# showlab/EgoVLP

Hardware: NVIDIA H100
Metric: clips/sec, 16-frame TimeSformer-B + DistilBERT + EgoNCE training step (higher is better)
Workload: dtype bf16

## Files before the change

### egovlp_b200/_lib.py

```python
import ctypes as C
import os

_PKG = os.path.dirname(os.path.abspath(__file__))
LIB_PATH = os.environ.get("EGOVLP_B200_LIB") or os.path.join(_PKG, "lib", "libegovlp_b200.so")
_lib = None


class GemmEpilogue(C.Structure):
    _fields_ = [("bias", C.c_void_p), ("residual", C.c_void_p), ("aux", C.c_void_p), ("out", C.c_void_p),
                ("out2", C.c_void_p), ("ldr", C.c_longlong), ("ldaux", C.c_longlong), ("ldo", C.c_longlong),
                ("ldo2", C.c_longlong), ("out_mode", C.c_int), ("act", C.c_int), ("alpha", C.c_float),
                ("col_scale", C.c_float), ("col_scale_ncols", C.c_int), ("res_row_mod", C.c_int), ("colsum", C.c_void_p),
                ("colsum_a", C.c_void_p), ("drop_p", C.c_float), ("drop_site", C.c_uint), ("drop_seed", C.c_ulonglong),
                ("path_p", C.c_float), ("path_site", C.c_uint), ("path_rows", C.c_int)]


class EgovlpError(RuntimeError):
    pass


def lib():
    global _lib
    if _lib is None:
        if not os.path.exists(LIB_PATH):
            raise EgovlpError(f"{LIB_PATH} is missing: build it with `python -m egovlp_b200.build` "
                              "(there is no CPU / PyTorch fallback for the hot path)")
        _lib = C.CDLL(LIB_PATH)
        _lib.egovlp_last_error.restype = C.c_char_p
        _lib.egovlp_divided_attn_workspace_floats.restype = C.c_longlong
        _lib.egovlp_egonce_fused_workspace_floats.restype = C.c_longlong
        _lib.egovlp_narrow_linear_workspace_floats.restype = C.c_longlong
        _lib.egovlp_space_attn_long_workspace_floats.restype = C.c_longlong
    return _lib


_KERNELS_PER_CALL = {"egovlp_egonce_fused_max_g": 0, "egovlp_divided_attn_fwd": 2, "egovlp_divided_attn_bwd": 2, "egovlp_video_embed_bwd": 2,
                     "egovlp_nce_fwd": 2, "egovlp_dual_softmax": 2, "egovlp_cross_entropy_fwd": 2,
                     "egovlp_narrow_linear_bwd": 3, "egovlp_text_attn_long_bwd": 3, "egovlp_space_attn_long_fwd": 2,
                     "egovlp_space_attn_long_bwd": 4}
_launches = 0


def reset_launch_count():
    global _launches
    _launches = 0


def launch_count():
    return _launches


def call(name, *args):
    global _launches
    fn = getattr(lib(), name)
    rc = fn(*args)
    _launches += _KERNELS_PER_CALL.get(name, 1)
    if rc != 0:
        raise EgovlpError(f"{name} failed ({rc}): {lib().egovlp_last_error().decode()}")


def declared_symbols():
    import re
# ... 5 lines not shown
```

### egovlp_b200/csrc/attention.cu

```cuda
#include <stdlib.h>

#include "common.cuh"
#include "egovlp_b200.h"

namespace egovlp {

bool space_attn_wgmma_supported(int N);
int space_attn_fwd_wgmma(const void* qkv, void* out, float* lse, float* cls_part, int B, int T, int N, int H,
                         cudaStream_t st);

namespace {

constexpr int HD = 64;
constexpr int ROW_BYTES = 128;
constexpr float LOG2E = 1.4426950408889634f;

struct Geom {
  int B, H, T, N, S, D;
  int mode;
  int PG;
  int G;
  int NP;
  int NPAD;
  int gsize;
};

__device__ __forceinline__ int row_token(const Geom& G, int g, int r) {
  if (r == G.NP) return 0;
  if (r > G.NP) return -1;
  if (G.mode == 1) return 1 + g * G.N + r;
  const int j = r / G.T, f = r - j * G.T, n = g * G.PG + j;
  return n < G.N ? 1 + f * G.N + n : -1;
}

template <int RT>
__device__ __forceinline__ int row_token_x(const Geom& G, int g, int r, int sh) {
  if (RT == 0) return row_token(G, g, r);
  if (r == G.NP) return 0;
  if (r > G.NP) return -1;
  if (RT == 1) return 1 + g * G.N + r;
  const int n = g * G.PG + (r >> sh);
  return n < G.N ? 1 + (r & ((1 << sh) - 1)) * G.N + n : -1;
}

struct Smem {
  uint32_t q, k, v, dout;
  short* gid;
  float* lse;
  float* delta;
  uint32_t stage;
  uint32_t bar;
};

__device__ __forceinline__ bool pair_valid(int gq, int gk, bool first_group) {
  if (gq >= 0) return gk == gq || gk == -2;
  if (gq == -2) return gk >= 0 || (gk == -2 && first_group);
  return false;
}

__device__ __forceinline__ void tile_window(const Geom& G, int r0, int& lo, int& hi) {
  if (r0 <= G.NP && G.NP < r0 + 16) { lo = 0; hi = G.NP; return; }
  if (r0 > G.NP) { lo = 0; hi = 0; return; }
  lo = (r0 / G.gsize) * G.gsize;
  hi = min(G.NP, ((r0 + 15) / G.gsize + 1) * G.gsize);
}
__device__ __forceinline__ bool span_active(const Geom& G, int lo, int hi, int c0, int width) {
  return (c0 < hi && c0 + width > lo) || (c0 <= G.NP && G.NP < c0 + width);
}

// ... 843 lines not shown
      }
      const float2 lq = *reinterpret_cast<const float2*>(sm.lse + col);
      const float2 dq2 = *reinterpret_cast<const float2*>(sm.delta + col);
      const f32x2 nl = pk2(-lq.x, -lq.y), nd = pk2(-dq2.x, -dq2.y);
      float e0, e1, e2, e3;
      up2(fma2(pk2(st[j][0], st[j][1]), sc, nl), e0, e1);
      up2(fma2(pk2(st[j][2], st[j][3]), sc, nl), e2, e3);
      const float p0 = exp2f(e0), p1 = exp2f(e1), p2 = exp2f(e2), p3 = exp2f(e3);
      pf[p][jj * 2] = pack_bf16x2(p0, p1);
      pf[p][jj * 2 + 1] = pack_bf16x2(p2, p3);
      float d0, d1, d2, d3;
      up2(mul2(pk2(p0, p1), add2(pk2(dpt[j][0], dpt[j][1]), nd)), d0, d1);
      up2(mul2(pk2(p2, p3), add2(pk2(dpt[j][2], dpt[j][3]), nd)), d2, d3);
      dsf[p][jj * 2] = pack_bf16x2(d0, d1);
      dsf[p][jj * 2 + 1] = pack_bf16x2(d2, d3);
    }
  }
#pragma unroll
  for (int p = 0; p < NPR; ++p) {
    const uint32_t qb = sm.q + ch.base[p] * ROW_BYTES, db = sm.dout + ch.base[p] * ROW_BYTES;
#pragma unroll
    for (int dpi = 0; dpi < 4; ++dpi) {
      uint32_t bf[4];
      ldsm_x4_t(db + fo.a[dpi], bf);
      mma_bf16(dv[2 * dpi], pf[p], bf[0], bf[1]);
      mma_bf16(dv[2 * dpi + 1], pf[p], bf[2], bf[3]);
      ldsm_x4_t(qb + fo.a[dpi], bf);
      mma_bf16(dk[2 * dpi], dsf[p], bf[0], bf[1]);
      mma_bf16(dk[2 * dpi + 1], dsf[p], bf[2], bf[3]);
    }
  }
}

template <bool TIME, int NWARPS, int MINB>
__global__ void __launch_bounds__(NWARPS * 32, MINB)
fast_attn_bwd_kernel(const __grid_constant__ CUtensorMap tm_qkv, const __grid_constant__ CUtensorMap tm_do,
                     const bf16* __restrict__ qkv, const bf16* __restrict__ out, const bf16* __restrict__ dout,
                     const float* __restrict__ lse_in, bf16* __restrict__ dqkv, float* __restrict__ dcls, float q_scale,
                     Geom G, int sh) {
  extern __shared__ uint8_t smem_raw[];
  const uint32_t smem_base = (smem_u32(smem_raw) + 1023u) & ~1023u;
  uint8_t* smem_gen = smem_raw + (smem_base - smem_u32(smem_raw));
  int b, h, g;
  decode_block(G, b, h, g);
  Smem sm;
  load_group<true, false, false, false>(G, &tm_qkv, &tm_do, qkv, dout, b, h, g, smem_gen, smem_base, sm, NWARPS);
  constexpr int RT = TIME ? 2 : 1;

  const int warp = threadIdx.x >> 5, lane = threadIdx.x & 31;
  const int gq = lane >> 2, t = lane & 3;
  FastCtx c;
  c.NP = G.NP; c.NPAD = G.NPAD; c.sh = sh; c.first_group = (g == 0);
  c.valid_keys = TIME ? min(G.PG, G.N - g * G.PG) * G.T : G.NP;
  const FragOff fo = make_frag_off(lane);

  constexpr int P0_ROWS = NWARPS * 4;
  constexpr int P0_MAX = (256 + P0_ROWS - 1) / P0_ROWS;
  constexpr int P0_N = TIME ? 128 / P0_ROWS : P0_MAX;
  uint4 o_pre[P0_N];
  float l_pre[P0_N];
  int t_pre[P0_N];
#pragma unroll
  for (int i = 0; i < P0_N; ++i) {
    const int r = warp * 4 + (lane >> 3) + i * P0_ROWS;
    const int tok = r < G.NPAD ? row_token_x<RT>(G, g, r, sh) : -1;
    t_pre[i] = tok;
    const int tc = max(tok, 0);
    o_pre[i] = __ldg(reinterpret_cast<const uint4*>(out + ((long long)b * G.S + tc) * G.D + h * HD + (lane & 7) * 8));
    l_pre[i] = __ldg(lse_in + ((long long)(b * G.H + h)) * G.S + tc);
  }
  mbar_wait(sm.bar, 0);
#pragma unroll
  for (int i = 0; i < P0_N; ++i) {
    const int r = warp * 4 + (lane >> 3) + i * P0_ROWS;
    if (r >= G.NPAD) break;
    const int tok = t_pre[i], cc = lane & 7;
    float d = 0.f;
    if (tok >= 0) {
      const uint4 ov = o_pre[i];
      const uint4 dv = *reinterpret_cast<const uint4*>(smem_gen + (sw_addr(sm.dout, r, cc) - smem_base));
      const uint32_t ou[4] = {ov.x, ov.y, ov.z, ov.w}, du[4] = {dv.x, dv.y, dv.z, dv.w};
#pragma unroll
      for (int i = 0; i < 4; ++i) {
        const float2 a = unpack_bf16x2(ou[i]), bb = unpack_bf16x2(du[i]);
        d += a.x * bb.x + a.y * bb.y;
      }
    }
    d += __shfl_xor_sync(0xffffffffu, d, 1); d += __shfl_xor_sync(0xffffffffu, d, 2); d += __shfl_xor_sync(0xffffffffu, d, 4);
    if (cc == 0) {
      sm.delta[r] = d;
      sm.lse[r] = tok >= 0 ? l_pre[i] * LOG2E : 0.f;
    }
  }
  __syncthreads();

  for (int it = warp;; it += NWARPS) {
    int r0, part;
    if (!work_item<TIME, NWARPS>(c, it, r0, part)) break;
    const int rowA = r0 + gq, rowB = rowA + 8;
    const float ls0 = sm.lse[rowA], ls1 = sm.lse[rowB], de0 = sm.delta[rowA], de1 = sm.delta[rowB];
    float dq[8][4];
#pragma unroll
    for (int j = 0; j < 8; ++j) { dq[j][0] = dq[j][1] = dq[j][2] = dq[j][3] = 0.f; }
    Chunk ch;
#pragma unroll 1
    for (int ci = 0; get_chunk<TIME, NWARPS, 2>(c, G.T, r0, part, ci, ch); ++ci) {
      if (ch.np == 2) bwd_q_chunk<TIME, 2>(c, sm, fo, ch, r0, rowA, rowB, t, ls0, ls1, de0, de1, dq);
      else bwd_q_chunk<TIME, 1>(c, sm, fo, ch, r0, rowA, rowB, t, ls0, ls1, de0, de1, dq);
    }
    {
      const int rc = c.NP - r0;
      if (rc >= 0 && rc < 16 && (rc & 7) == gq) {
        const bool hi_half = rc >= 8;
        float* dst = dcls + ((long long)(b * G.H + h) * 3 + 0) * HD;
#pragma unroll
        for (int j = 0; j < 8; ++j) {
          atomicAdd(dst + j * 8 + 2 * t, hi_half ? dq[j][2] : dq[j][0]);
          atomicAdd(dst + j * 8 + 2 * t + 1, hi_half ? dq[j][3] : dq[j][1]);
        }
      }
    }
    if (part < 0) store_frag_rows_bf16<RT>(dq, q_scale, dqkv, 3 * G.D, h * HD, G, b, g, r0, lane, -1.f, sh);
  }

  for (int it = warp;; it += NWARPS) {
    int k0r, part;
    if (!work_item<TIME, NWARPS>(c, it, k0r, part)) break;
    const int keyA = k0r + gq, keyB = keyA + 8;
    float dk[8][4], dv[8][4];
#pragma unroll
    for (int j = 0; j < 8; ++j) { dk[j][0] = dk[j][1] = dk[j][2] = dk[j][3] = 0.f; dv[j][0] = dv[j][1] = dv[j][2] = dv[j][3] = 0.f; }
    Chunk ch;
#pragma unroll 1
    for (int ci = 0; get_chunk<TIME, NWARPS, 2>(c, G.T, k0r, part, ci, ch); ++ci) {
      if (ch.np == 2) bwd_k_chunk<TIME, 2>(c, sm, fo, ch, k0r, keyA, keyB, t, dk, dv);
      else bwd_k_chunk<TIME, 1>(c, sm, fo, ch, k0r, keyA, keyB, t, dk, dv);
    }
    {
      const int rc = c.NP - k0r;
      if (rc >= 0 && rc < 16 && (rc & 7) == gq) {
        const bool hi_half = rc >= 8;
        float* dstk = dcls + ((long long)(b * G.H + h) * 3 + 1) * HD;
        float* dstv = dcls + ((long long)(b * G.H + h) * 3 + 2) * HD;
#pragma unroll
        for (int j = 0; j < 8; ++j) {
          atomicAdd(dstk + j * 8 + 2 * t, hi_half ? dk[j][2] : dk[j][0]);
          atomicAdd(dstk + j * 8 + 2 * t + 1, hi_half ? dk[j][3] : dk[j][1]);
          atomicAdd(dstv + j * 8 + 2 * t, hi_half ? dv[j][2] : dv[j][0]);
          atomicAdd(dstv + j * 8 + 2 * t + 1, hi_half ? dv[j][3] : dv[j][1]);
        }
      }
    }
    if (part < 0) {
      store_frag_rows_bf16<RT>(dk, 1.f, dqkv, 3 * G.D, G.D + h * HD, G, b, g, k0r, lane, -1.f, sh);
      store_frag_rows_bf16<RT>(dv, 1.f, dqkv, 3 * G.D, 2 * G.D + h * HD, G, b, g, k0r, lane, -1.f, sh);
    }
  }
}

inline bool force_generic() {
  const char* e = getenv("EGOVLP_ATTN_GENERIC");
  return e && e[0] == '1';
}
inline bool time_fast_ok(const Geom& G) { return G.mode == 0 && (G.T == 4 || G.T == 8 || G.T == 16) && G.NP == 112; }
inline int time_shift(const Geom& G) { return G.T == 16 ? 4 : G.T == 8 ? 3 : 2; }

int make_geom(Geom& G, int B, int T, int N, int H, int mode) {
  G.B = B; G.H = H; G.T = T; G.N = N; G.S = 1 + T * N; G.D = H * HD; G.mode = mode;
  if (mode == 1) {
    G.PG = N; G.G = T; G.NP = N; G.gsize = N;
  } else {
    G.PG = (T <= 16 && 16 % T == 0) ? min(N, 112 / T) : min(N, 127 / T);
    if (G.PG < 1) return EGOVLP_ERR_UNSUPPORTED;
    G.G = (N + G.PG - 1) / G.PG; G.NP = G.PG * T; G.gsize = T;
  }
  G.NPAD = (G.NP + 1 + 15) / 16 * 16;
  if (G.NPAD > 256 || (mode == 1 ? N : max(T, G.PG)) > 256) return EGOVLP_ERR_UNSUPPORTED;
  return EGOVLP_OK;
}

int make_group_tmap(CUtensorMap* tm, const void* base, const Geom& G, int ncolblk) {
  const uint64_t W = (uint64_t)ncolblk * HD;
  const uint64_t dims[5] = {HD, (uint64_t)G.T, (uint64_t)G.N, (uint64_t)ncolblk, (uint64_t)G.B};
  const uint64_t strides[5] = {1, (uint64_t)G.N * W, W, HD, (uint64_t)G.S * W};
  const uint32_t box[5] = {HD, (uint32_t)(G.mode == 1 ? 1 : G.T), (uint32_t)(G.mode == 1 ? G.N : G.PG), 1, 1};
  return make_tmap_nd_bf16(tm, reinterpret_cast<const bf16*>(base) + W, 5, dims, strides, box, true);
}

size_t attn_smem_bytes(const Geom& G, bool bwd, int nwarps, bool staging = true) {
  return (size_t)(bwd ? 4 : 3) * G.NPAD * ROW_BYTES + ((bwd || !staging) ? 0 : nwarps * 16 * ROW_BYTES) + 2 * G.NPAD * 4 +
// ... 11 lines not shown
  if (make_geom(G, B, T, N, H, mode)) return -1;
  return (long long)B * H * G.G * 4 * 66;
}

extern "C" int egovlp_divided_attn_fwd(const void* qkv, void* out, float* lse, float* cls_part, int B, int T, int N,
                                       int H, int mode, void* stream) {
  EGOVLP_CHECK_ARG(qkv && out && lse && cls_part, "divided_attn_fwd: null pointer");
  EGOVLP_CHECK_ARG(B > 0 && T > 0 && N > 0 && H > 0 && (mode == 0 || mode == 1), "divided_attn_fwd: bad shape");
  Geom G;
  if (make_geom(G, B, T, N, H, mode)) { set_last_error("divided_attn: unsupported geometry T=%d N=%d", T, N); return EGOVLP_ERR_UNSUPPORTED; }
  CUtensorMap tm;
  int rc = make_group_tmap(&tm, qkv, G, 3 * H);
  if (rc) return rc;
  cudaStream_t st = reinterpret_cast<cudaStream_t>(stream);
  const bf16* q = reinterpret_cast<const bf16*>(qkv);
  bf16* o = reinterpret_cast<bf16*>(out);
  const int grid = B * H * G.G;
#define LAUNCH_FWD(KERN, W, ...)                                                                              \
  do {                                                                                                        \
    const size_t smem = attn_smem_bytes(G, false, W, generic || mode == 1);                                   \
    EGOVLP_CHECK_CUDA(cudaFuncSetAttribute(KERN, cudaFuncAttributeMaxDynamicSharedMemorySize, (int)smem));    \
    KERN<<<grid, W * 32, smem, st>>>(tm, q, o, lse, cls_part, G, ##__VA_ARGS__);                              \
  } while (0)
  const bool generic = force_generic() || (mode == 0 && !time_fast_ok(G));
  if (!generic && mode == 1 && space_attn_wgmma_supported(N)) {
    rc = space_attn_fwd_wgmma(qkv, out, lse, cls_part, B, T, N, H, st);
    if (rc) return rc;
  } else if (generic) {
    if (G.NPAD > 128) LAUNCH_FWD((divided_attn_fwd_kernel<7, 2>), 7);
    else LAUNCH_FWD((divided_attn_fwd_kernel<4, 3>), 4);
  } else if (mode == 1) {
    if (G.NPAD > 128) LAUNCH_FWD((fast_attn_fwd_kernel<false, 7, 2>), 7, 0);
    else LAUNCH_FWD((fast_attn_fwd_kernel<false, 4, 3>), 4, 0);
  } else {
    LAUNCH_FWD((fast_attn_fwd_kernel<true, 4, 4>), 4, time_shift(G));
  }
#undef LAUNCH_FWD
  EGOVLP_CHECK_LAUNCH();
  const int BH = B * H;
  const int parts = (!generic && mode == 0) ? 4 : 1;
  cls_merge_kernel<<<(BH + 3) / 4, 128, 0, st>>>(cls_part, o, lse, BH, H, G.G * parts, G.S, G.D);
  EGOVLP_CHECK_LAUNCH();
  return EGOVLP_OK;
}

extern "C" int egovlp_divided_attn_bwd(const void* qkv, const void* out, const void* dout, const float* lse,
                                       void* dqkv, float* dcls_ws, int B, int T, int N, int H, int mode,
                                       float q_scale, void* stream) {
  EGOVLP_CHECK_ARG(qkv && out && dout && lse && dqkv && dcls_ws, "divided_attn_bwd: null pointer");
  EGOVLP_CHECK_ARG(B > 0 && T > 0 && N > 0 && H > 0 && (mode == 0 || mode == 1), "divided_attn_bwd: bad shape");
  Geom G;
  if (make_geom(G, B, T, N, H, mode)) { set_last_error("divided_attn: unsupported geometry T=%d N=%d", T, N); return EGOVLP_ERR_UNSUPPORTED; }
  CUtensorMap tmq, tmd;
  int rc = make_group_tmap(&tmq, qkv, G, 3 * H);
  if (rc) return rc;
  rc = make_group_tmap(&tmd, dout, G, H);
  if (rc) return rc;
  cudaStream_t st = reinterpret_cast<cudaStream_t>(stream);
  EGOVLP_CHECK_CUDA(cudaMemsetAsync(dcls_ws, 0, (size_t)B * H * 3 * HD * sizeof(float), st));
  const bf16* q = reinterpret_cast<const bf16*>(qkv);
  const bf16* o = reinterpret_cast<const bf16*>(out);
  const bf16* d_o = reinterpret_cast<const bf16*>(dout);
  bf16* dq = reinterpret_cast<bf16*>(dqkv);
  const int grid = B * H * G.G;
#define LAUNCH_BWD(KERN, W, ...)                                                                              \
  do {                                                                                                        \
    const size_t smem = attn_smem_bytes(G, true, W);                                                          \
    EGOVLP_CHECK_CUDA(cudaFuncSetAttribute(KERN, cudaFuncAttributeMaxDynamicSharedMemorySize, (int)smem));    \
    KERN<<<grid, W * 32, smem, st>>>(tmq, tmd, q, o, d_o, lse, dq, dcls_ws, q_scale, G, ##__VA_ARGS__);       \
  } while (0)
  const bool generic = force_generic() || (mode == 0 && !time_fast_ok(G));
  if (generic) {
    if (G.NPAD > 128) LAUNCH_BWD((divided_attn_bwd_kernel<7, 2>), 7);
    else LAUNCH_BWD((divided_attn_bwd_kernel<4, 3>), 4);
  } else if (mode == 1) {
    if (G.NPAD > 128) LAUNCH_BWD((fast_attn_bwd_kernel<false, 7, 2>), 7, 0);
    else LAUNCH_BWD((fast_attn_bwd_kernel<false, 4, 3>), 4, 0);
  } else {
    const char* we = getenv("EGOVLP_ATTN_TIME_BWD_WARPS");
    const bool w8 = we && we[0] == '8';
    if (w8) LAUNCH_BWD((fast_attn_bwd_kernel<true, 8, 2>), 8, time_shift(G));
    else LAUNCH_BWD((fast_attn_bwd_kernel<true, 4, 3>), 4, time_shift(G));
  }
#undef LAUNCH_BWD
  EGOVLP_CHECK_LAUNCH();
  const int n = B * H * 3 * HD;
  cls_grad_finalize_kernel<<<(n + 255) / 256, 256, 0, st>>>(dcls_ws, reinterpret_cast<bf16*>(dqkv), B, H, G.S, G.D, q_scale);
  EGOVLP_CHECK_LAUNCH();
  return EGOVLP_OK;
}
```

### egovlp_b200/csrc/common.cuh

```cuda
#pragma once
#include <cuda.h>
#include <cuda_bf16.h>
#include <cuda_runtime.h>
#include <stdint.h>
#include <stdio.h>

#define EGOVLP_OK 0
#define EGOVLP_ERR_ARG (-1)
#define EGOVLP_ERR_CUDA (-2)
#define EGOVLP_ERR_UNSUPPORTED (-3)

namespace egovlp {

typedef __nv_bfloat16 bf16;

void set_last_error(const char* fmt, ...);

#define EGOVLP_CHECK_ARG(cond, ...)                                   \
  do {                                                                \
    if (!(cond)) {                                                    \
      ::egovlp::set_last_error(__VA_ARGS__);                          \
      return EGOVLP_ERR_ARG;                                          \
    }                                                                 \
  } while (0)
// ... 181 lines not shown
  asm volatile(
      "cp.async.bulk.tensor.4d.shared::cluster.global.mbarrier::complete_tx::bytes [%0], [%1, {%3, %4, %5, %6}], [%2];"
      ::"r"(dst), "l"(reinterpret_cast<uint64_t>(m)), "r"(bar), "r"(c0), "r"(c1), "r"(c2), "r"(c3)
      : "memory");
}
__device__ __forceinline__ void tma_load_5d(uint32_t dst, const CUtensorMap* m, uint32_t bar, int c0, int c1, int c2,
                                            int c3, int c4) {
  asm volatile(
      "cp.async.bulk.tensor.5d.shared::cluster.global.mbarrier::complete_tx::bytes [%0], [%1, {%3, %4, %5, %6, %7}], [%2];"
      ::"r"(dst), "l"(reinterpret_cast<uint64_t>(m)), "r"(bar), "r"(c0), "r"(c1), "r"(c2), "r"(c3), "r"(c4)
      : "memory");
}
__device__ __forceinline__ void tma_load_2d_multicast(uint32_t dst, const CUtensorMap* m, uint32_t bar, int c0, int c1,
                                                      uint16_t mask) {
  asm volatile(
      "cp.async.bulk.tensor.2d.shared::cluster.global.mbarrier::complete_tx::bytes.multicast::cluster"
      " [%0], [%1, {%3, %4}], [%2], %5;"
      ::"r"(dst), "l"(reinterpret_cast<uint64_t>(m)), "r"(bar), "r"(c0), "r"(c1), "h"(mask)
      : "memory");
}
__device__ __forceinline__ void fence_proxy_async_smem() {
  asm volatile("fence.proxy.async.shared::cta;" ::: "memory");
}
__device__ __forceinline__ void bulk_load_1d(uint32_t dst, const void* src, uint32_t bytes, uint32_t bar) {
  asm volatile("cp.async.bulk.shared::cluster.global.mbarrier::complete_tx::bytes [%0], [%1], %2, [%3];"
               ::"r"(dst), "l"(reinterpret_cast<uint64_t>(src)), "r"(bytes), "r"(bar)
               : "memory");
}
__device__ __forceinline__ void tma_store_2d(const CUtensorMap* m, uint32_t src, int c0, int c1) {
  asm volatile("cp.async.bulk.tensor.2d.global.shared::cta.bulk_group [%0, {%2, %3}], [%1];"
               ::"l"(reinterpret_cast<uint64_t>(m)), "r"(src), "r"(c0), "r"(c1)
               : "memory");
}
__device__ __forceinline__ void tma_reduce_add_2d(const CUtensorMap* m, uint32_t src, int c0, int c1) {
  asm volatile("cp.reduce.async.bulk.tensor.2d.global.shared::cta.add.tile.bulk_group [%0, {%2, %3}], [%1];"
               ::"l"(reinterpret_cast<uint64_t>(m)), "r"(src), "r"(c0), "r"(c1)
               : "memory");
}
__device__ __forceinline__ void bulk_commit() { asm volatile("cp.async.bulk.commit_group;" ::: "memory"); }
template <int N>
__device__ __forceinline__ void bulk_wait_read() { asm volatile("cp.async.bulk.wait_group.read %0;" ::"n"(N) : "memory"); }
template <int N>
__device__ __forceinline__ void bulk_wait() { asm volatile("cp.async.bulk.wait_group %0;" ::"n"(N) : "memory"); }
__device__ __forceinline__ void named_bar_sync(int id, int count) {
  asm volatile("bar.sync %0, %1;" ::"r"(id), "r"(count) : "memory");
}

__device__ __forceinline__ uint32_t cluster_ctarank() {
  uint32_t r;
  asm volatile("mov.u32 %0, %%cluster_ctarank;" : "=r"(r));
  return r;
}
__device__ __forceinline__ void cluster_sync_all() {
  asm volatile("barrier.cluster.arrive.release.aligned;\n\tbarrier.cluster.wait.acquire.aligned;" ::: "memory");
}
__device__ __forceinline__ uint32_t mapa_shared(uint32_t addr, uint32_t cta_rank) {
  uint32_t r;
  asm volatile("mapa.shared::cluster.u32 %0, %1, %2;" : "=r"(r) : "r"(addr), "r"(cta_rank));
  return r;
}
__device__ __forceinline__ void mbar_arrive_cluster(uint32_t cluster_addr) {
  asm volatile("mbarrier.arrive.release.cluster.shared::cluster.b64 _, [%0];" ::"r"(cluster_addr) : "memory");
}

__device__ __forceinline__ void wgmma_fence() { asm volatile("wgmma.fence.sync.aligned;" ::: "memory"); }
__device__ __forceinline__ void wgmma_commit() { asm volatile("wgmma.commit_group.sync.aligned;" ::: "memory"); }
// ... 28 lines not shown
```

### egovlp_b200/ops.py

```python
import ctypes as C

import torch

from ._lib import GemmEpilogue, call, lib

BF16, F32, E4M3 = torch.bfloat16, torch.float32, torch.float8_e4m3fn


def _ptr(t):
    return C.c_void_p(t.data_ptr()) if t is not None else C.c_void_p(0)


def _stream():
    return C.c_void_p(torch.cuda.current_stream().cuda_stream)


def _chk(t, dtype, name):
    assert t.is_cuda and t.dtype == dtype, f"{name}: expected cuda {dtype}, got {t.device} {t.dtype}"


_prof = None


def profile(enable):
# ... 183 lines not shown
    return raw, torch.tensor(ct, dtype=torch.int32, device=dev), torch.tensor(co, dtype=torch.int32, device=dev)


def cast_multi(raw, chunk_tensor, chunk_offset):
    call("egovlp_cast_multi_f32_to_bf16", _ptr(raw), _ptr(chunk_tensor), _ptr(chunk_offset), chunk_tensor.numel(),
         _stream())


def colsum_accum(dy, out):
    assert dy.dim() == 2 and dy.stride(1) == 1 and out.dtype == F32 and out.numel() == dy.shape[1]
    call("egovlp_colsum_accum", _ptr(dy), int(dy.dtype == F32), C.c_longlong(dy.stride(0)), _ptr(out), dy.shape[0],
         dy.shape[1], _stream())


def divided_attn_fwd(qkv, B, T, N, H, mode):
    _chk(qkv, BF16, "qkv")
    S, D = 1 + T * N, 64 * H
    assert qkv.is_contiguous() and qkv.shape == (B * S, 3 * D)
    out = torch.empty(B * S, D, dtype=BF16, device=qkv.device)
    lse = torch.empty(B, H, S, dtype=F32, device=qkv.device)
    n_ws = lib().egovlp_divided_attn_workspace_floats(B, T, N, H, mode)
    assert n_ws > 0, "unsupported attention geometry"
    ws = torch.empty(n_ws, dtype=F32, device=qkv.device)
    with _Probe("attn_time_fwd" if mode == 0 else "attn_space_fwd", B * S * (8 * D + 4 * H)):
        call("egovlp_divided_attn_fwd", _ptr(qkv), _ptr(out), _ptr(lse), _ptr(ws), B, T, N, H, mode, _stream())
    return out, lse


def divided_attn_bwd(qkv, out, dout, lse, B, T, N, H, mode, q_scale, dqkv=None):
    _chk(qkv, BF16, "qkv"); _chk(out, BF16, "out"); _chk(dout, BF16, "dout"); _chk(lse, F32, "lse")
    assert qkv.is_contiguous() and out.is_contiguous() and dout.is_contiguous() and lse.is_contiguous()
    if dqkv is None:
        dqkv = torch.empty_like(qkv)
    ws = torch.empty(B * H * 3 * 64, dtype=F32, device=qkv.device)
    S, D = 1 + T * N, 64 * H
    with _Probe("attn_time_bwd" if mode == 0 else "attn_space_bwd", B * S * (16 * D + 4 * H)):
        call("egovlp_divided_attn_bwd", _ptr(qkv), _ptr(out), _ptr(dout), _ptr(lse), _ptr(dqkv), _ptr(ws), B, T, N, H,
             mode, C.c_float(q_scale), _stream())
    return dqkv


def _space_long_ws(B, T, N, H, device):
    n_ws = lib().egovlp_space_attn_long_workspace_floats(B, T, N, H)
    assert n_ws > 0, f"space_attn_long: unsupported geometry B={B} T={T} N={N} H={H}"
    return torch.empty(n_ws, dtype=F32, device=device)


def space_attn_long_fwd(qkv, B, T, N, H):
    _chk(qkv, BF16, "qkv")
    S, D = 1 + T * N, 64 * H
    assert qkv.is_contiguous() and qkv.shape == (B * S, 3 * D)
    out = torch.empty(B * S, D, dtype=BF16, device=qkv.device)
    lse = torch.empty(B, H, S, dtype=F32, device=qkv.device)
    ws = _space_long_ws(B, T, N, H, qkv.device)
    with _Probe("attn_space_long_fwd", B * S * (8 * D + 4 * H)):
        call("egovlp_space_attn_long_fwd", _ptr(qkv), _ptr(out), _ptr(lse), _ptr(ws), B, T, N, H, _stream())
    return out, lse


def space_attn_long_bwd(qkv, out, dout, lse, B, T, N, H, q_scale, dqkv=None):
    _chk(qkv, BF16, "qkv"); _chk(out, BF16, "out"); _chk(dout, BF16, "dout"); _chk(lse, F32, "lse")
    assert qkv.is_contiguous() and out.is_contiguous() and dout.is_contiguous() and lse.is_contiguous()
    if dqkv is None:
        dqkv = torch.empty_like(qkv)
    S, D = 1 + T * N, 64 * H
    ws = _space_long_ws(B, T, N, H, qkv.device)
    with _Probe("attn_space_long_bwd", B * S * (16 * D + 4 * H)):
# ... 418 lines not shown
```

### include/egovlp_b200.h

```cpp
#ifndef EGOVLP_B200_H_
#define EGOVLP_B200_H_

#include <stdint.h>

#ifdef __cplusplus
extern "C" {
#endif

#define EGOVLP_ERR_ARG (-1)
#define EGOVLP_ERR_CUDA (-2)
#define EGOVLP_ERR_UNSUPPORTED (-3)

const char* egovlp_last_error(void);
int egovlp_abi_version(void);

typedef struct egovlp_gemm_epilogue {
  const float* bias;
  const float* residual;
  const void* aux;
  void* out;
  void* out2;
  long long ldr, ldaux, ldo, ldo2;
  int out_mode;
  int act;
  float alpha;
  float col_scale;
  int col_scale_ncols;
  int res_row_mod;
  float* colsum;
  float* colsum_a;
  float drop_p;
  unsigned int drop_site;
  unsigned long long drop_seed;
  float path_p;
  unsigned int path_site;
  int path_rows;
} egovlp_gemm_epilogue;

int egovlp_gemm_bf16(const void* A, int a_mn_major, long long lda, const void* B, int b_mn_major, long long ldb,
                     int M, int N, int K, const egovlp_gemm_epilogue* epi, int split_k, void* stream);
int egovlp_gemm_e4m3(const void* A8, long long lda, const void* B8, long long ldb, const float* row_scale,
                     const float* col_scale, int M, int N, int K, const egovlp_gemm_epilogue* epi, void* stream);

int egovlp_layernorm_fwd(const float* x, long long ldx, const float* add, float* sum_out, const float* gamma,
                         const float* beta, void* y_bf16, float* y_f32, float* mean, float* rstd, int rows, int D,
                         float eps, void* stream);
int egovlp_layernorm_fwd_e4m3(const float* x, long long ldx, const float* gamma, const float* beta, void* y_bf16,
                              float* y_f32, float* mean, float* rstd, uint8_t* y8, float* row_scale, int rows, int D,
                              float eps, void* stream);
int egovlp_layernorm_bwd(const void* dy, int dy_is_bf16, long long lddy, const float* x, long long ldx,
                         const float* gamma, const float* mean, const float* rstd, const void* add1, int add1_is_bf16,
                         const void* add2, int add2_is_bf16, float* dx, long long lddx, void* dx_bf16, float* dgamma,
                         float* dbeta, float* colsum_dx, int rows, int D, void* stream);

long long egovlp_divided_attn_workspace_floats(int B, int T, int N, int H, int mode);
int egovlp_divided_attn_fwd(const void* qkv, void* out, float* lse, float* cls_part, int B, int T, int N, int H,
                            int mode, void* stream);
int egovlp_divided_attn_bwd(const void* qkv, const void* out, const void* dout, const float* lse, void* dqkv,
                            float* dcls_ws, int B, int T, int N, int H, int mode, float q_scale, void* stream);
long long egovlp_space_attn_long_workspace_floats(int B, int T, int N, int H);
int egovlp_space_attn_long_fwd(const void* qkv, void* out, float* lse, float* workspace, int B, int T, int N, int H,
                               void* stream);
int egovlp_space_attn_long_bwd(const void* qkv, const void* out, const void* dout, const float* lse, void* dqkv,
                               float* workspace, int B, int T, int N, int H, float q_scale, void* stream);

int egovlp_patch_im2col(const float* video, void* patches_bf16, int B, int T, int C, int H, int W, int P, void* stream);
int egovlp_patch_im2col_u8(const uint8_t* video, void* patches_bf16, int B, int T, int C, int H, int W, int P,
                           const float* host_mean3, const float* host_std3, void* stream);
int egovlp_video_transform_max_taps(void);
int egovlp_video_transform_max_res(void);
int egovlp_video_transform(const uint8_t* frames, long long frames_bytes, const long long* desc, int B, int F, int R,
                           int center_crop, const float* host_mean, const float* host_std, float* out, void* stream);
int egovlp_video_pos_table(const float* cls_token, const float* pos_embed, const float* temporal_embed,
                           const float* conv_bias, float* table, int T, int N, int D, void* stream);
int egovlp_video_embed_bwd(const float* dx, float* tmp_SD, float* dcls, float* dpos, float* dtemporal, float* dbias,
                           int B, int T, int N, int D, void* stream);

int egovlp_text_embed_fwd(const long long* input_ids, const float* word_emb, const float* pos_emb, float* out, int B,
                          int L, int D, void* stream);
int egovlp_text_embed_bwd(const long long* input_ids, const float* dsum, float* dword, float* dpos, int B, int L, int D,
                          void* stream);
int egovlp_text_attn_fwd(const void* qkv, const long long* attention_mask, void* out, int B, int L, int H, float p_drop,
                         unsigned long long seed, unsigned int site, void* stream);
int egovlp_text_attn_bwd(const void* qkv, const long long* attention_mask, const void* dout, void* dqkv, int B, int L,
                         int H, float q_scale, float p_drop, unsigned long long seed, unsigned int site, void* stream);
int egovlp_text_attn_long_fwd(const void* qkv, const long long* attention_mask, void* out, float* lse, int B, int L,
                              int H, float p_drop, unsigned long long seed, unsigned int site, void* stream);
int egovlp_text_attn_long_bwd(const void* qkv, const long long* attention_mask, const void* out, const float* lse,
// ... 99 lines not shown
```

Before: 184.2.

## Add persistent TMA-pipelined time-attention forward and backward kernels for T=16

Adds dedicated persistent kernels for temporal attention with 16 frames. They loop over (batch, head, group) items and double-buffer (forward) or prefetch (backward) Q/K/V/dO tiles via TMA, with the CLS row loaded separately. The forward kernel writes its output through a TMA store. The backward kernel replaces the zeroed global CLS-gradient workspace with per-group partials, which a small finalize kernel then reduces. The generic fast backward kernel is de-templated to handle space attention only. The changes target launch and tail overhead and the exposed load latency of one-CTA-per-group kernels, at the cost of a larger workspace, one extra kernel launch, and more code paths.

```diff
diff --git a/egovlp_b200/_lib.py b/egovlp_b200/_lib.py
--- a/egovlp_b200/_lib.py
+++ b/egovlp_b200/_lib.py
@@ -28,6 +28,7 @@
         _lib = C.CDLL(LIB_PATH)
         _lib.egovlp_last_error.restype = C.c_char_p
         _lib.egovlp_divided_attn_workspace_floats.restype = C.c_longlong
+        _lib.egovlp_divided_attn_bwd_workspace_floats.restype = C.c_longlong
         _lib.egovlp_egonce_fused_workspace_floats.restype = C.c_longlong
         _lib.egovlp_narrow_linear_workspace_floats.restype = C.c_longlong
         _lib.egovlp_space_attn_long_workspace_floats.restype = C.c_longlong
diff --git a/egovlp_b200/csrc/attention.cu b/egovlp_b200/csrc/attention.cu
--- a/egovlp_b200/csrc/attention.cu
+++ b/egovlp_b200/csrc/attention.cu
@@ -34,7 +34,7 @@
 }
 
 template <int RT>
-__device__ __forceinline__ int row_token_x(const Geom& G, int g, int r, int sh) {
+__device__ __forceinline__ int row_token_x(const Geom& G, int g, int r, int sh = 0) {
   if (RT == 0) return row_token(G, g, r);
   if (r == G.NP) return 0;
   if (r > G.NP) return -1;
@@ -944,12 +944,12 @@
   }
 }
 
-template <bool TIME, int NWARPS, int MINB>
+template <int NWARPS, int MINB>
 __global__ void __launch_bounds__(NWARPS * 32, MINB)
 fast_attn_bwd_kernel(const __grid_constant__ CUtensorMap tm_qkv, const __grid_constant__ CUtensorMap tm_do,
                      const bf16* __restrict__ qkv, const bf16* __restrict__ out, const bf16* __restrict__ dout,
                      const float* __restrict__ lse_in, bf16* __restrict__ dqkv, float* __restrict__ dcls, float q_scale,
-                     Geom G, int sh) {
+                     Geom G) {
   extern __shared__ uint8_t smem_raw[];
   const uint32_t smem_base = (smem_u32(smem_raw) + 1023u) & ~1023u;
   uint8_t* smem_gen = smem_raw + (smem_base - smem_u32(smem_raw));
@@ -957,25 +957,24 @@
   decode_block(G, b, h, g);
   Smem sm;
   load_group<true, false, false, false>(G, &tm_qkv, &tm_do, qkv, dout, b, h, g, smem_gen, smem_base, sm, NWARPS);
-  constexpr int RT = TIME ? 2 : 1;
 
   const int warp = threadIdx.x >> 5, lane = threadIdx.x & 31;
   const int gq = lane >> 2, t = lane & 3;
   FastCtx c;
-  c.NP = G.NP; c.NPAD = G.NPAD; c.sh = sh; c.first_group = (g == 0);
-  c.valid_keys = TIME ? min(G.PG, G.N - g * G.PG) * G.T : G.NP;
+  c.NP = G.NP; c.NPAD = G.NPAD; c.sh = 0; c.first_group = (g == 0);
+  c.valid_keys = G.NP;
   const FragOff fo = make_frag_off(lane);
 
   constexpr int P0_ROWS = NWARPS * 4;
   constexpr int P0_MAX = (256 + P0_ROWS - 1) / P0_ROWS;
-  constexpr int P0_N = TIME ? 128 / P0_ROWS : P0_MAX;
+  constexpr int P0_N = P0_MAX;
   uint4 o_pre[P0_N];
   float l_pre[P0_N];
   int t_pre[P0_N];
 #pragma unroll
   for (int i = 0; i < P0_N; ++i) {
     const int r = warp * 4 + (lane >> 3) + i * P0_ROWS;
-    const int tok = r < G.NPAD ? row_token_x<RT>(G, g, r, sh) : -1;
+    const int tok = r < G.NPAD ? row_token_x<1>(G, g, r) : -1;
     t_pre[i] = tok;
     const int tc = max(tok, 0);
     o_pre[i] = __ldg(reinterpret_cast<const uint4*>(out + ((long long)b * G.S + tc) * G.D + h * HD + (lane & 7) * 8));
@@ -1008,7 +1007,7 @@
 
   for (int it = warp;; it += NWARPS) {
     int r0, part;
-    if (!work_item<TIME, NWARPS>(c, it, r0, part)) break;
+    if (!work_item<false, NWARPS>(c, it, r0, part)) break;
     const int rowA = r0 + gq, rowB = rowA + 8;
     const float ls0 = sm.lse[rowA], ls1 = sm.lse[rowB], de0 = sm.delta[rowA], de1 = sm.delta[rowB];
     float dq[8][4];
@@ -1016,9 +1015,9 @@
     for (int j = 0; j < 8; ++j) { dq[j][0] = dq[j][1] = dq[j][2] = dq[j][3] = 0.f; }
     Chunk ch;
 #pragma unroll 1
-    for (int ci = 0; get_chunk<TIME, NWARPS, 2>(c, G.T, r0, part, ci, ch); ++ci) {
-      if (ch.np == 2) bwd_q_chunk<TIME, 2>(c, sm, fo, ch, r0, rowA, rowB, t, ls0, ls1, de0, de1, dq);
-      else bwd_q_chunk<TIME, 1>(c, sm, fo, ch, r0, rowA, rowB, t, ls0, ls1, de0, de1, dq);
+    for (int ci = 0; get_chunk<false, NWARPS, 2>(c, G.T, r0, part, ci, ch); ++ci) {
+      if (ch.np == 2) bwd_q_chunk<false, 2>(c, sm, fo, ch, r0, rowA, rowB, t, ls0, ls1, de0, de1, dq);
+      else bwd_q_chunk<false, 1>(c, sm, fo, ch, r0, rowA, rowB, t, ls0, ls1, de0, de1, dq);
     }
     {
       const int rc = c.NP - r0;
@@ -1032,21 +1031,21 @@
         }
       }
     }
-    if (part < 0) store_frag_rows_bf16<RT>(dq, q_scale, dqkv, 3 * G.D, h * HD, G, b, g, r0, lane, -1.f, sh);
+    store_frag_rows_bf16<1>(dq, q_scale, dqkv, 3 * G.D, h * HD, G, b, g, r0, lane);
   }
 
   for (int it = warp;; it += NWARPS) {
     int k0r, part;
-    if (!work_item<TIME, NWARPS>(c, it, k0r, part)) break;
+    if (!work_item<false, NWARPS>(c, it, k0r, part)) break;
     const int keyA = k0r + gq, keyB = keyA + 8;
     float dk[8][4], dv[8][4];
 #pragma unroll
     for (int j = 0; j < 8; ++j) { dk[j][0] = dk[j][1] = dk[j][2] = dk[j][3] = 0.f; dv[j][0] = dv[j][1] = dv[j][2] = dv[j][3] = 0.f; }
     Chunk ch;
 #pragma unroll 1
-    for (int ci = 0; get_chunk<TIME, NWARPS, 2>(c, G.T, k0r, part, ci, ch); ++ci) {
-      if (ch.np == 2) bwd_k_chunk<TIME, 2>(c, sm, fo, ch, k0r, keyA, keyB, t, dk, dv);
-      else bwd_k_chunk<TIME, 1>(c, sm, fo, ch, k0r, keyA, keyB, t, dk, dv);
+    for (int ci = 0; get_chunk<false, NWARPS, 2>(c, G.T, k0r, part, ci, ch); ++ci) {
+      if (ch.np == 2) bwd_k_chunk<false, 2>(c, sm, fo, ch, k0r, keyA, keyB, t, dk, dv);
+      else bwd_k_chunk<false, 1>(c, sm, fo, ch, k0r, keyA, keyB, t, dk, dv);
     }
     {
       const int rc = c.NP - k0r;
@@ -1063,11 +1062,308 @@
         }
       }
     }
-    if (part < 0) {
-      store_frag_rows_bf16<RT>(dk, 1.f, dqkv, 3 * G.D, G.D + h * HD, G, b, g, k0r, lane, -1.f, sh);
-      store_frag_rows_bf16<RT>(dv, 1.f, dqkv, 3 * G.D, 2 * G.D + h * HD, G, b, g, k0r, lane, -1.f, sh);
-    }
-  }
+    store_frag_rows_bf16<1>(dk, 1.f, dqkv, 3 * G.D, G.D + h * HD, G, b, g, k0r, lane);
+    store_frag_rows_bf16<1>(dv, 1.f, dqkv, 3 * G.D, 2 * G.D + h * HD, G, b, g, k0r, lane);
+  }
+}
+
+constexpr int TIME_BWD_STAGES = 1;
+constexpr int TIME_BWD_WARPS = 4;
+constexpr int TIME_BWD_CTAS = 3;
+constexpr int TIME_BWD_PARTS = 4;
+constexpr int TIME_NPAD = 128;
+
+__device__ __forceinline__ void time_item(const Geom& G, int i, int& b, int& h, int& g) {
+  h = i % G.H;
+  const int bg = i / G.H;
+  g = bg % G.G;
+  b = bg / G.G;
+}
+
+template <int NTILES>
+__device__ __forceinline__ void time_issue_loads(const Geom& G, const CUtensorMap* tm_qkv, const CUtensorMap* tm_qkv_row,
+                                                 const CUtensorMap* tm_do, const CUtensorMap* tm_do_row, uint32_t st,
+                                                 uint32_t bar, int b, int h, int g) {
+  const uint32_t tile = TIME_NPAD * ROW_BYTES, cls = G.NP * ROW_BYTES;
+  mbar_expect_tx(bar, (uint32_t)(NTILES * (G.NP + 1) * ROW_BYTES));
+#pragma unroll
+  for (int w = 0; w < 3; ++w) {
+    tma_load_5d(st + w * tile, tm_qkv, bar, 0, 0, g * G.PG, w * G.H + h, b);
+    tma_load_2d(st + w * tile + cls, tm_qkv_row, bar, w * G.D + h * HD, b * G.S);
+  }
+  if (NTILES == 4) {
+    tma_load_5d(st + 3 * tile, tm_do, bar, 0, 0, g * G.PG, h, b);
+    tma_load_2d(st + 3 * tile + cls, tm_do_row, bar, h * HD, b * G.S);
+  }
+}
+
+__device__ __forceinline__ void time_zero_padding(uint8_t* smem_gen, int NP, int ntiles) {
+  const int pad = TIME_NPAD - NP - 1;
+  for (int i = threadIdx.x; i < ntiles * pad * 8; i += blockDim.x) {
+    const int c = i & 7, r = NP + 1 + (i >> 3) % pad, tl = (i >> 3) / pad;
+    *reinterpret_cast<uint4*>(smem_gen + sw_addr(tl * TIME_NPAD * ROW_BYTES, r, c)) = make_uint4(0, 0, 0, 0);
+  }
+}
+
+constexpr int TIME_FWD_STAGES = 2;
+constexpr int TIME_FWD_WARPS = 8;
+constexpr int TIME_FWD_PARTS = 4;
+
+__global__ void __launch_bounds__(TIME_FWD_WARPS * 32, 2)
+time_attn_fwd_kernel(const __grid_constant__ CUtensorMap tm_qkv, const __grid_constant__ CUtensorMap tm_qkv_row,
+                     const __grid_constant__ CUtensorMap tm_out, float* __restrict__ lse_out,
+                     float* __restrict__ cls_part, Geom G, int sh, int n_items) {
+  constexpr int NW = TIME_FWD_WARPS, PARTS = TIME_FWD_PARTS;
+  constexpr uint32_t TILE = TIME_NPAD * ROW_BYTES, STAGE = 3 * TILE;
+  extern __shared__ uint8_t smem_raw[];
+  const uint32_t smem_base = (smem_u32(smem_raw) + 1023u) & ~1023u;
+  uint8_t* smem_gen = smem_raw + (smem_base - smem_u32(smem_raw));
+  const uint32_t bar0 = smem_base + TIME_FWD_STAGES * STAGE;
+  const int tid = threadIdx.x, warp = tid >> 5, lane = tid & 31, gq = lane >> 2, t = lane & 3;
+  time_zero_padding(smem_gen, G.NP, TIME_FWD_STAGES * 3);
+  if (tid == 0) {
+    for (int s = 0; s < TIME_FWD_STAGES; ++s) mbar_init(bar0 + 8 * s, 1);
+    fence_mbar_init();
+    for (int s = 0; s < TIME_FWD_STAGES; ++s) {
+      const int i = blockIdx.x + s * gridDim.x;
+      if (i >= n_items) break;
+      int b, h, g;
+      time_item(G, i, b, h, g);
+      time_issue_loads<3>(G, &tm_qkv, &tm_qkv_row, nullptr, nullptr, smem_base + s * STAGE, bar0 + 8 * s, b, h, g);
+    }
+  }
+  __syncthreads();
+  const FragOff fo = make_frag_off(lane);
+
+#pragma unroll 1
+  for (int k = 0, i = blockIdx.x; i < n_items; ++k, i += gridDim.x) {
+    const int s = k % TIME_FWD_STAGES;
+    int b, h, g;
+    time_item(G, i, b, h, g);
+    Smem sm;
+    sm.q = smem_base + s * STAGE;
+    sm.k = sm.q + TILE;
+    sm.v = sm.k + TILE;
+    FastCtx c;
+    c.NP = G.NP; c.NPAD = TIME_NPAD; c.sh = sh; c.first_group = (g == 0);
+    c.valid_keys = min(G.PG, G.N - g * G.PG) * G.T;
+    mbar_wait(bar0 + 8 * s, (k / TIME_FWD_STAGES) & 1);
+
+    for (int it = warp;; it += NW) {
+      int r0, part;
+      if (!work_item<true, PARTS>(c, it, r0, part)) break;
+      const int rowA = r0 + gq, rowB = rowA + 8;
+      uint32_t qf[4][4];
+#pragma unroll
+      for (int kk = 0; kk < 4; ++kk) ldsm_x4(sm.q + r0 * ROW_BYTES + fo.a[kk], qf[kk]);
+      float m0 = -INFINITY, m1 = -INFINITY, l0 = 0.f, l1 = 0.f;
+      float o[8][4];
+#pragma unroll
+      for (int j = 0; j < 8; ++j) { o[j][0] = o[j][1] = o[j][2] = o[j][3] = 0.f; }
+      Chunk ch;
+      get_chunk<true, PARTS, 4>(c, G.T, r0, part, 0, ch);
+      fwd_chunk<true, 2>(c, sm, fo, ch, qf, rowA, rowB, t, m0, m1, l0, l1, o);
+      l0 += __shfl_xor_sync(0xffffffffu, l0, 1); l0 += __shfl_xor_sync(0xffffffffu, l0, 2);
+      l1 += __shfl_xor_sync(0xffffffffu, l1, 1); l1 += __shfl_xor_sync(0xffffffffu, l1, 2);
+      if (part >= 0) {
+        if (gq == 0) {
+          float* dst = cls_part + ((((long long)(b * G.H + h)) * G.G + g) * PARTS + part) * 66;
+#pragma unroll
+          for (int j = 0; j < 8; ++j) *reinterpret_cast<float2*>(dst + j * 8 + 2 * t) = make_float2(o[j][0], o[j][1]);
+          if (t == 0) { dst[64] = m0; dst[65] = l0; }
+        }
+        continue;
+      }
+      const float i0 = l0 > 0.f ? 1.f / l0 : 0.f, i1 = l1 > 0.f ? 1.f / l1 : 0.f;
+      if (t == 0) {
+        const int tok0 = row_token_x<2>(G, g, rowA, sh), tok1 = row_token_x<2>(G, g, rowB, sh);
+        if (tok0 > 0) lse_out[((long long)(b * G.H + h)) * G.S + tok0] = m0 + logf(l0);
+        if (tok1 > 0) lse_out[((long long)(b * G.H + h)) * G.S + tok1] = m1 + logf(l1);
+      }
+#pragma unroll
+      for (int j = 0; j < 8; ++j) {
+        asm volatile("st.shared.b32 [%0], %1;" ::"r"(sw_addr(sm.q, rowA, j) + t * 4), "r"(pack_bf16x2(o[j][0] * i0, o[j][1] * i0)));
+        asm volatile("st.shared.b32 [%0], %1;" ::"r"(sw_addr(sm.q, rowB, j) + t * 4), "r"(pack_bf16x2(o[j][2] * i1, o[j][3] * i1)));
+      }
+    }
+    fence_proxy_async_smem();
+    __syncthreads();
+    if (tid == 0) {
+      tma_store_5d(&tm_out, sm.q, 0, 0, g * G.PG, h, b);
+      bulk_commit();
+      const int nx = i + TIME_FWD_STAGES * gridDim.x;
+      if (nx < n_items) {
+        bulk_wait_read<0>();
+        int nb, nh, ng;
+        time_item(G, nx, nb, nh, ng);
+        time_issue_loads<3>(G, &tm_qkv, &tm_qkv_row, nullptr, nullptr, sm.q, bar0 + 8 * s, nb, nh, ng);
+      }
+    }
+  }
+  if (tid == 0) bulk_wait<0>();
+}
+
+__global__ void __launch_bounds__(TIME_BWD_WARPS * 32, TIME_BWD_CTAS)
+time_attn_bwd_kernel(const __grid_constant__ CUtensorMap tm_qkv, const __grid_constant__ CUtensorMap tm_qkv_row,
+                     const __grid_constant__ CUtensorMap tm_do, const __grid_constant__ CUtensorMap tm_do_row,
+                     const bf16* __restrict__ out, const float* __restrict__ lse_in, bf16* __restrict__ dqkv,
+                     float* __restrict__ dcls_part, float q_scale, Geom G, int sh, int n_items) {
+  constexpr int NW = TIME_BWD_WARPS, PARTS = TIME_BWD_PARTS;
+  constexpr uint32_t TILE = TIME_NPAD * ROW_BYTES, STAGE = 4 * TILE;
+  constexpr int P0_ROWS = NW * 4;
+  constexpr int P0_N = (TIME_NPAD + P0_ROWS - 1) / P0_ROWS;
+  extern __shared__ uint8_t smem_raw[];
+  const uint32_t smem_base = (smem_u32(smem_raw) + 1023u) & ~1023u;
+  uint8_t* smem_gen = smem_raw + (smem_base - smem_u32(smem_raw));
+  float* s_lse = reinterpret_cast<float*>(smem_gen + TIME_BWD_STAGES * STAGE);
+  float* s_delta = s_lse + TIME_NPAD;
+  float* s_cls = s_delta + TIME_NPAD;
+  const uint32_t bar0 = smem_base + TIME_BWD_STAGES * STAGE + (2 * TIME_NPAD + PARTS * 3 * HD) * 4;
+
+  const int tid = threadIdx.x, warp = tid >> 5, lane = tid & 31, gq = lane >> 2, t = lane & 3;
+  time_zero_padding(smem_gen, G.NP, TIME_BWD_STAGES * 4);
+  if (tid == 0) {
+    for (int s = 0; s < TIME_BWD_STAGES; ++s) mbar_init(bar0 + 8 * s, 1);
+    fence_mbar_init();
+    for (int s = 0; s < TIME_BWD_STAGES; ++s) {
+      const int i = blockIdx.x + s * gridDim.x;
+      if (i >= n_items) break;
+      int b, h, g;
+      time_item(G, i, b, h, g);
+      time_issue_loads<4>(G, &tm_qkv, &tm_qkv_row, &tm_do, &tm_do_row, smem_base + s * STAGE, bar0 + 8 * s, b, h, g);
+    }
+  }
+  __syncthreads();
+
+  uint4 o_pre[P0_N];
+  float l_pre[P0_N];
+  auto prefetch = [&](int i) {
+    if (i >= n_items) return;
+    int b, h, g;
+    time_item(G, i, b, h, g);
+#pragma unroll
+    for (int j = 0; j < P0_N; ++j) {
+      const int tc = max(row_token_x<2>(G, g, warp * 4 + (lane >> 3) + j * P0_ROWS, sh), 0);
+      o_pre[j] = __ldg(reinterpret_cast<const uint4*>(out + ((long long)b * G.S + tc) * G.D + h * HD + (lane & 7) * 8));
+      l_pre[j] = __ldg(lse_in + ((long long)(b * G.H + h)) * G.S + tc);
+    }
+  };
+  prefetch(blockIdx.x);
+  const FragOff fo = make_frag_off(lane);
+
+#pragma unroll 1
+  for (int k = 0, i = blockIdx.x; i < n_items; ++k, i += gridDim.x) {
+    const int s = k % TIME_BWD_STAGES;
+    int b, h, g;
+    time_item(G, i, b, h, g);
+    Smem sm;
+    sm.q = smem_base + s * STAGE;
+    sm.k = sm.q + TILE;
+    sm.v = sm.k + TILE;
+    sm.dout = sm.v + TILE;
+    sm.lse = s_lse;
+    sm.delta = s_delta;
+    FastCtx c;
+    c.NP = G.NP; c.NPAD = TIME_NPAD; c.sh = sh; c.first_group = (g == 0);
+    c.valid_keys = min(G.PG, G.N - g * G.PG) * G.T;
+    mbar_wait(bar0 + 8 * s, (k / TIME_BWD_STAGES) & 1);
+
+#pragma unroll
+    for (int j = 0; j < P0_N; ++j) {
+      const int r = warp * 4 + (lane >> 3) + j * P0_ROWS, cc = lane & 7;
+      if (r >= TIME_NPAD) break;
+      const int tok = row_token_x<2>(G, g, r, sh);
+      float d = 0.f;
+      if (tok >= 0) {
+        const uint4 ov = o_pre[j];
+        const uint4 dv = *reinterpret_cast<const uint4*>(smem_gen + (sw_addr(sm.dout, r, cc) - smem_base));
+        const uint32_t ou[4] = {ov.x, ov.y, ov.z, ov.w}, du[4] = {dv.x, dv.y, dv.z, dv.w};
+#pragma unroll
+        for (int e = 0; e < 4; ++e) {
+          const float2 a = unpack_bf16x2(ou[e]), bb = unpack_bf16x2(du[e]);
+          d += a.x * bb.x + a.y * bb.y;
+        }
+      }
+      d += __shfl_xor_sync(0xffffffffu, d, 1); d += __shfl_xor_sync(0xffffffffu, d, 2); d += __shfl_xor_sync(0xffffffffu, d, 4);
+      if (cc == 0) {
+        s_delta[r] = d;
+        s_lse[r] = tok >= 0 ? l_pre[j] * LOG2E : 0.f;
+      }
+    }
+    prefetch(i + gridDim.x);
+    __syncthreads();
+
+    for (int it = warp;; it += NW) {
+      int r0, part;
+      if (!work_item<true, PARTS>(c, it, r0, part)) break;
+      const int rowA = r0 + gq, rowB = rowA + 8;
+      const float ls0 = s_lse[rowA], ls1 = s_lse[rowB], de0 = s_delta[rowA], de1 = s_delta[rowB];
+      float dq[8][4];
+#pragma unroll
+      for (int j = 0; j < 8; ++j) { dq[j][0] = dq[j][1] = dq[j][2] = dq[j][3] = 0.f; }
+      Chunk ch;
+      get_chunk<true, PARTS, 2>(c, G.T, r0, part, 0, ch);
+      bwd_q_chunk<true, 2>(c, sm, fo, ch, r0, rowA, rowB, t, ls0, ls1, de0, de1, dq);
+      if (part >= 0) {
+        if (gq == 0) {
+#pragma unroll
+          for (int j = 0; j < 8; ++j) *reinterpret_cast<float2*>(s_cls + (part * 3 + 0) * HD + j * 8 + 2 * t) = make_float2(dq[j][0], dq[j][1]);
+        }
+      } else {
+        store_frag_rows_bf16<2>(dq, q_scale, dqkv, 3 * G.D, h * HD, G, b, g, r0, lane, -1.f, sh);
+      }
+    }
+
+    for (int it = warp;; it += NW) {
+      int k0r, part;
+      if (!work_item<true, PARTS>(c, it, k0r, part)) break;
+      const int keyA = k0r + gq, keyB = keyA + 8;
+      float dk[8][4], dv[8][4];
+#pragma unroll
+      for (int j = 0; j < 8; ++j) { dk[j][0] = dk[j][1] = dk[j][2] = dk[j][3] = 0.f; dv[j][0] = dv[j][1] = dv[j][2] = dv[j][3] = 0.f; }
+      Chunk ch;
+      get_chunk<true, PARTS, 2>(c, G.T, k0r, part, 0, ch);
+      bwd_k_chunk<true, 2>(c, sm, fo, ch, k0r, keyA, keyB, t, dk, dv);
+      if (part >= 0) {
+        if (gq == 0) {
+#pragma unroll
+          for (int j = 0; j < 8; ++j) {
+            *reinterpret_cast<float2*>(s_cls + (part * 3 + 1) * HD + j * 8 + 2 * t) = make_float2(dk[j][0], dk[j][1]);
+            *reinterpret_cast<float2*>(s_cls + (part * 3 + 2) * HD + j * 8 + 2 * t) = make_float2(dv[j][0], dv[j][1]);
+          }
+        }
+      } else {
+        store_frag_rows_bf16<2>(dk, 1.f, dqkv, 3 * G.D, G.D + h * HD, G, b, g, k0r, lane, -1.f, sh);
+        store_frag_rows_bf16<2>(dv, 1.f, dqkv, 3 * G.D, 2 * G.D + h * HD, G, b, g, k0r, lane, -1.f, sh);
+      }
+    }
+    __syncthreads();
+    if (tid == 0) {
+      const int nx = i + TIME_BWD_STAGES * gridDim.x;
+      if (nx < n_items) {
+        int nb, nh, ng;
+        time_item(G, nx, nb, nh, ng);
+        time_issue_loads<4>(G, &tm_qkv, &tm_qkv_row, &tm_do, &tm_do_row, sm.q, bar0 + 8 * s, nb, nh, ng);
+      }
+    }
+    for (int e = tid; e < 3 * HD; e += NW * 32) {
+      float acc = 0.f;
+#pragma unroll
+      for (int p = 0; p < PARTS; ++p) acc += s_cls[p * 3 * HD + e];
+      dcls_part[((long long)(b * G.H + h) * G.G + g) * 3 * HD + e] = acc;
+    }
+  }
+}
+
+__global__ void time_cls_grad_finalize_kernel(const float* __restrict__ part, bf16* __restrict__ dqkv, int B, int H,
+                                              int Gn, int S, int D, float q_scale) {
+  const int i = blockIdx.x * blockDim.x + threadIdx.x;
+  if (i >= B * H * 3 * HD) return;
+  const int e = i % (3 * HD), bh = i / (3 * HD), d = e % HD, which = e / HD, h = bh % H, b = bh / H;
+  const float* p = part + (long long)bh * Gn * 3 * HD + e;
+  float acc = 0.f;
+  for (int g = 0; g < Gn; ++g) acc += p[(long long)g * 3 * HD];
+  dqkv[(long long)b * S * 3 * D + which * D + h * HD + d] = __float2bfloat16(acc * (which == 0 ? q_scale : 1.f));
 }
 
 inline bool force_generic() {
@@ -1145,6 +1441,17 @@
   } else if (mode == 1) {
     if (G.NPAD > 128) LAUNCH_FWD((fast_attn_fwd_kernel<false, 7, 2>), 7, 0);
     else LAUNCH_FWD((fast_attn_fwd_kernel<false, 4, 3>), 4, 0);
+  } else if (G.T == 16) {
+    CUtensorMap tm_row, tm_out;
+    rc = make_tmap_2d_bf16(&tm_row, qkv, (uint64_t)B * G.S, 3 * G.D, 3 * G.D, 1, HD);
+    if (rc) return rc;
+    rc = make_group_tmap(&tm_out, out, G, H);
+    if (rc) return rc;
+    const size_t smem = (size_t)TIME_FWD_STAGES * 3 * TIME_NPAD * ROW_BYTES + 8 * TIME_FWD_STAGES + 1024;
+    EGOVLP_CHECK_CUDA(cudaFuncSetAttribute(time_attn_fwd_kernel, cudaFuncAttributeMaxDynamicSharedMemorySize, (int)smem));
+    const int n_items = B * H * G.G;
+    time_attn_fwd_kernel<<<min(n_items, 2 * num_sms()), TIME_FWD_WARPS * 32, smem, st>>>(tm, tm_row, tm_out, lse,
+                                                                                          cls_part, G, time_shift(G), n_items);
   } else {
     LAUNCH_FWD((fast_attn_fwd_kernel<true, 4, 4>), 4, time_shift(G));
   }
@@ -1155,6 +1462,12 @@
   cls_merge_kernel<<<(BH + 3) / 4, 128, 0, st>>>(cls_part, o, lse, BH, H, G.G * parts, G.S, G.D);
   EGOVLP_CHECK_LAUNCH();
   return EGOVLP_OK;
+}
+
+extern "C" long long egovlp_divided_attn_bwd_workspace_floats(int B, int T, int N, int H, int mode) {
+  Geom G;
+  if (make_geom(G, B, T, N, H, mode)) return -1;
+  return (long long)B * H * (time_fast_ok(G) ? G.G : 1) * 3 * HD;
 }
 
 extern "C" int egovlp_divided_attn_bwd(const void* qkv, const void* out, const void* dout, const float* lse,
@@ -1170,11 +1483,30 @@
   rc = make_group_tmap(&tmd, dout, G, H);
   if (rc) return rc;
   cudaStream_t st = reinterpret_cast<cudaStream_t>(stream);
-  EGOVLP_CHECK_CUDA(cudaMemsetAsync(dcls_ws, 0, (size_t)B * H * 3 * HD * sizeof(float), st));
   const bf16* q = reinterpret_cast<const bf16*>(qkv);
   const bf16* o = reinterpret_cast<const bf16*>(out);
   const bf16* d_o = reinterpret_cast<const bf16*>(dout);
   bf16* dq = reinterpret_cast<bf16*>(dqkv);
+  const bool generic = force_generic() || (mode == 0 && !time_fast_ok(G));
+  if (!generic && mode == 0) {
+    CUtensorMap tmq_row, tmd_row;
+    rc = make_tmap_2d_bf16(&tmq_row, qkv, (uint64_t)B * G.S, 3 * G.D, 3 * G.D, 1, HD);
+    if (rc) return rc;
+    rc = make_tmap_2d_bf16(&tmd_row, dout, (uint64_t)B * G.S, G.D, G.D, 1, HD);
+    if (rc) return rc;
+    const size_t smem = (size_t)TIME_BWD_STAGES * 4 * TIME_NPAD * ROW_BYTES + (2 * TIME_NPAD + TIME_BWD_PARTS * 3 * HD) * 4 +
+                        8 * TIME_BWD_STAGES + 1024;
+    EGOVLP_CHECK_CUDA(cudaFuncSetAttribute(time_attn_bwd_kernel, cudaFuncAttributeMaxDynamicSharedMemorySize, (int)smem));
+    const int n_items = B * H * G.G;
+    time_attn_bwd_kernel<<<min(n_items, TIME_BWD_CTAS * num_sms()), TIME_BWD_WARPS * 32, smem, st>>>(
+        tmq, tmq_row, tmd, tmd_row, o, lse, dq, dcls_ws, q_scale, G, time_shift(G), n_items);
+    EGOVLP_CHECK_LAUNCH();
+    const int n = B * H * 3 * HD;
+    time_cls_grad_finalize_kernel<<<(n + 255) / 256, 256, 0, st>>>(dcls_ws, dq, B, H, G.G, G.S, G.D, q_scale);
+    EGOVLP_CHECK_LAUNCH();
+    return EGOVLP_OK;
+  }
+  EGOVLP_CHECK_CUDA(cudaMemsetAsync(dcls_ws, 0, (size_t)B * H * 3 * HD * sizeof(float), st));
   const int grid = B * H * G.G;
 #define LAUNCH_BWD(KERN, W, ...)                                                                              \
   do {                                                                                                        \
@@ -1182,18 +1514,12 @@
     EGOVLP_CHECK_CUDA(cudaFuncSetAttribute(KERN, cudaFuncAttributeMaxDynamicSharedMemorySize, (int)smem));    \
     KERN<<<grid, W * 32, smem, st>>>(tmq, tmd, q, o, d_o, lse, dq, dcls_ws, q_scale, G, ##__VA_ARGS__);       \
   } while (0)
-  const bool generic = force_generic() || (mode == 0 && !time_fast_ok(G));
   if (generic) {
     if (G.NPAD > 128) LAUNCH_BWD((divided_attn_bwd_kernel<7, 2>), 7);
     else LAUNCH_BWD((divided_attn_bwd_kernel<4, 3>), 4);
-  } else if (mode == 1) {
-    if (G.NPAD > 128) LAUNCH_BWD((fast_attn_bwd_kernel<false, 7, 2>), 7, 0);
-    else LAUNCH_BWD((fast_attn_bwd_kernel<false, 4, 3>), 4, 0);
   } else {
-    const char* we = getenv("EGOVLP_ATTN_TIME_BWD_WARPS");
-    const bool w8 = we && we[0] == '8';
-    if (w8) LAUNCH_BWD((fast_attn_bwd_kernel<true, 8, 2>), 8, time_shift(G));
-    else LAUNCH_BWD((fast_attn_bwd_kernel<true, 4, 3>), 4, time_shift(G));
+    if (G.NPAD > 128) LAUNCH_BWD((fast_attn_bwd_kernel<7, 2>), 7);
+    else LAUNCH_BWD((fast_attn_bwd_kernel<4, 3>), 4);
   }
 #undef LAUNCH_BWD
   EGOVLP_CHECK_LAUNCH();
diff --git a/egovlp_b200/csrc/common.cuh b/egovlp_b200/csrc/common.cuh
--- a/egovlp_b200/csrc/common.cuh
+++ b/egovlp_b200/csrc/common.cuh
@@ -237,6 +237,11 @@
                ::"l"(reinterpret_cast<uint64_t>(m)), "r"(src), "r"(c0), "r"(c1)
                : "memory");
 }
+__device__ __forceinline__ void tma_store_5d(const CUtensorMap* m, uint32_t src, int c0, int c1, int c2, int c3, int c4) {
+  asm volatile("cp.async.bulk.tensor.5d.global.shared::cta.bulk_group [%0, {%2, %3, %4, %5, %6}], [%1];"
+               ::"l"(reinterpret_cast<uint64_t>(m)), "r"(src), "r"(c0), "r"(c1), "r"(c2), "r"(c3), "r"(c4)
+               : "memory");
+}
 __device__ __forceinline__ void tma_reduce_add_2d(const CUtensorMap* m, uint32_t src, int c0, int c1) {
   asm volatile("cp.reduce.async.bulk.tensor.2d.global.shared::cta.add.tile.bulk_group [%0, {%2, %3}], [%1];"
                ::"l"(reinterpret_cast<uint64_t>(m)), "r"(src), "r"(c0), "r"(c1)
diff --git a/egovlp_b200/ops.py b/egovlp_b200/ops.py
--- a/egovlp_b200/ops.py
+++ b/egovlp_b200/ops.py
@@ -239,7 +239,9 @@
     assert qkv.is_contiguous() and out.is_contiguous() and dout.is_contiguous() and lse.is_contiguous()
     if dqkv is None:
         dqkv = torch.empty_like(qkv)
-    ws = torch.empty(B * H * 3 * 64, dtype=F32, device=qkv.device)
+    n_ws = lib().egovlp_divided_attn_bwd_workspace_floats(B, T, N, H, mode)
+    assert n_ws > 0, "unsupported attention geometry"
+    ws = torch.empty(n_ws, dtype=F32, device=qkv.device)
     S, D = 1 + T * N, 64 * H
     with _Probe("attn_time_bwd" if mode == 0 else "attn_space_bwd", B * S * (16 * D + 4 * H)):
         call("egovlp_divided_attn_bwd", _ptr(qkv), _ptr(out), _ptr(dout), _ptr(lse), _ptr(dqkv), _ptr(ws), B, T, N, H,
diff --git a/include/egovlp_b200.h b/include/egovlp_b200.h
--- a/include/egovlp_b200.h
+++ b/include/egovlp_b200.h
@@ -54,6 +54,7 @@
                          float* dbeta, float* colsum_dx, int rows, int D, void* stream);
 
 long long egovlp_divided_attn_workspace_floats(int B, int T, int N, int H, int mode);
+long long egovlp_divided_attn_bwd_workspace_floats(int B, int T, int N, int H, int mode);
 int egovlp_divided_attn_fwd(const void* qkv, void* out, float* lse, float* cls_part, int B, int T, int N, int H,
                             int mode, void* stream);
 int egovlp_divided_attn_bwd(const void* qkv, const void* out, const void* dout, const float* lse, void* dqkv,
```

Result: no change. 184.4 (median of 6 runs) (+0.1%).
